# hby1320/pytorch_object_detection

Measured on AMD Instinct MI355X. Metric: images/sec HISFCOS-R50 640x640 inference, higher is better.
Workload: dtype f32

## Files before the change

include/fcosdet.h:

```cpp
#ifndef FCOSDET_H_
#define FCOSDET_H_

#include <stdint.h>

#ifdef __cplusplus
extern "C" {
#endif

#define FD_OK 0
#define FD_E_INVAL (-1)
#define FD_E_UNSUPPORTED (-2)
#define FD_E_LAUNCH (-3)

#define FD_MAX_SEG 8

#define FD_ACT_NONE 0
#define FD_ACT_RELU 1
#define FD_ACT_SILU 2
#define FD_ACT_EXP 3
#define FD_ACT_SIGMOID 4

typedef void* fd_stream_t;

typedef struct fd_segs {
// ... 55 lines not shown
    void* workspace;
    int64_t workspace_bytes;
    int32_t precision;
    int32_t res_mode;
    float seg_param[FD_MAX_SEG];
    fd_segs in;
    int32_t out_H, out_W;
    int32_t sc_sy, sc_sx, sc_oy, sc_ox, sc_H, sc_W;
    const float* gate;
    int32_t gate_cs;
    int32_t reserved0;
    const float* w_frag;
    float* gn_stats;
    int32_t gn_groups;
    int32_t gate_act;
    const float* gate_b;
    const float* x2;
    int32_t x2_cs, x2_co, x2_Cin, x2_stride, x2_H, x2_W;
    int32_t wg_first, wg_count;
    int32_t sk_wgs;
    int32_t io_f16;
} fd_conv_params;
int64_t fd_conv_sk_workspace_bytes(int32_t sk_wgs);

int32_t fd_conv2d_nhwc_f32(const fd_conv_params* p, fd_stream_t stream);
int32_t fd_conv_workgroups(const fd_conv_params* p);
int32_t fd_conv_workgroups_live(const fd_conv_params* p);
typedef struct fd_b2b_params {
    const float* x; const float* w1_frag; const float* scale1; const float* shift1; const float* res; float* y;
    const float* w2_frag; const float* scale2; const float* shift2; float* z;
    int32_t x_cs, x_co, res_cs, res_co, y_cs, y_co, z_cs, z_co;
    int32_t K1, N1, N2, act1, act2, reserved0;
    int64_t rows;
} fd_b2b_params;
int32_t fd_conv1x1_b2b_f32(const fd_b2b_params* p, fd_stream_t stream);
int32_t fd_conv_narrow_nco(int32_t Cout);
int64_t fd_conv_workspace_bytes(int64_t out_rows, int32_t Cout, int32_t ksplit);

int64_t fd_wino4_weight_bytes(int32_t N, int32_t K);
int32_t fd_wino4_pack_weights_f32(const float* w, const float* scale, float* out, int32_t Cout, int32_t Cin, int32_t mode, fd_stream_t stream);

int64_t fd_conv_weight_wave_bytes(int32_t Cout, int32_t Cin);
int32_t fd_pack_conv_weight_wave_f32(const float* w, float* out, int32_t Cout, int32_t Cin, fd_stream_t stream);

int64_t fd_wino_weight_bytes(int32_t Cout, int32_t Cin);
int32_t fd_wino_pack_weights_f32(const float* w, const float* scale, float* out, int32_t Cout, int32_t Cin, int32_t mode,
                                 fd_stream_t stream);

typedef struct fd_conv_wgrad_params {
    const float* x;
    const float* dy;
    float* dw;
    int32_t x_cs, x_co, dy_cs, dy_co;
    int32_t Cin, Cout, KH, KW, stride, pad, dil;
    void* workspace;
    int64_t workspace_bytes;
    int32_t nsplit;
    int32_t layout;
    const float* scale;
    fd_segs in;
    int32_t precision;
    int32_t io_f16;
} fd_conv_wgrad_params;

int64_t fd_conv_wgrad_workspace_bytes(int64_t out_rows, int32_t Cin, int32_t Cout, int32_t KH, int32_t KW);
int32_t fd_conv2d_bwd_weight_f32(const fd_conv_wgrad_params* p, fd_stream_t stream);
// ... 239 lines not shown
```

pytorch_object_detection_amd/_lib.py:

```python
from __future__ import annotations

import ctypes as C
import os

FD_MAX_SEG = 8
ACT_NONE, ACT_RELU, ACT_SILU, ACT_EXP, ACT_SIGMOID = 0, 1, 2, 3, 4
CONV_GENERIC, CONV_STEM = 0, 1
PREC_F32, PREC_F16X3, PREC_F16 = 0, 1, 2
TILES = {1: (128, 128), 2: (128, 64), 3: (64, 128), 4: (64, 64), 5: (128, 32), 6: (128, 96),
         7: (128, 128), 8: (128, 64), 9: (64, 128),
         10: (256, 128), 11: (256, 128),
         12: (128, 96),
         13: (128, 128),
         15: (64, 64)}
PATCH_TILE = 13
WAVE_TILE = 15
WINO_TILE = 14
WINO4_TILE = 16
NARROW_TILE = 17
F16K64_TILE = 18

_HERE = os.path.dirname(os.path.abspath(__file__))
LIB_PATH = os.environ.get("FD_LIB") or os.path.join(_HERE, "csrc", "libfcosdet_hip.so")

# ... 8 lines not shown
E_INVAL, E_UNSUPPORTED, E_LAUNCH = -1, -2, -3


class Segs(C.Structure):
    _fields_ = [("nseg", C.c_int32), ("batch", C.c_int32), ("H", C.c_int32 * FD_MAX_SEG), ("W", C.c_int32 * FD_MAX_SEG),
                ("m_start", C.c_int32 * (FD_MAX_SEG + 1))]

    @staticmethod
    def make(batch: int, hw) -> "Segs":
        s = Segs()
        s.nseg, s.batch = len(hw), batch
        m = 0
        for i, (h, w) in enumerate(hw):
            s.H[i], s.W[i], s.m_start[i] = h, w, m
            m += batch * h * w
        for i in range(len(hw), FD_MAX_SEG + 1):
            s.m_start[i] = m
        return s

    @property
    def rows(self) -> int:
        return self.m_start[self.nseg]

    def level_hw(self):
        return [(self.H[i], self.W[i]) for i in range(self.nseg)]


class B2BParams(C.Structure):
    _fields_ = [("x", C.c_void_p), ("w1_frag", C.c_void_p), ("scale1", C.c_void_p), ("shift1", C.c_void_p), ("res", C.c_void_p), ("y", C.c_void_p),
                ("w2_frag", C.c_void_p), ("scale2", C.c_void_p), ("shift2", C.c_void_p), ("z", C.c_void_p),
                ("x_cs", C.c_int32), ("x_co", C.c_int32), ("res_cs", C.c_int32), ("res_co", C.c_int32), ("y_cs", C.c_int32), ("y_co", C.c_int32),
                ("z_cs", C.c_int32), ("z_co", C.c_int32),
                ("K1", C.c_int32), ("N1", C.c_int32), ("N2", C.c_int32), ("act1", C.c_int32), ("act2", C.c_int32), ("reserved0", C.c_int32),
                ("rows", C.c_int64)]


class ConvParams(C.Structure):
    _fields_ = [("x", C.c_void_p), ("w", C.c_void_p), ("scale", C.c_void_p), ("shift", C.c_void_p), ("res", C.c_void_p),
                ("y", C.c_void_p),
                ("x_cs", C.c_int32), ("x_co", C.c_int32), ("res_cs", C.c_int32), ("res_co", C.c_int32),
                ("y_cs", C.c_int32), ("y_co", C.c_int32),
                ("Cin", C.c_int32), ("Cout", C.c_int32), ("KH", C.c_int32), ("KW", C.c_int32), ("stride", C.c_int32),
                ("pad", C.c_int32), ("dil", C.c_int32),
                ("act", C.c_int32), ("act_c0", C.c_int32), ("mode", C.c_int32), ("tile", C.c_int32), ("tag", C.c_int32), ("ksplit", C.c_int32),
                ("workspace", C.c_void_p), ("workspace_bytes", C.c_int64), ("precision", C.c_int32), ("res_mode", C.c_int32),
                ("seg_param", C.c_float * FD_MAX_SEG), ("segs", Segs),
                ("out_H", C.c_int32), ("out_W", C.c_int32), ("sc_sy", C.c_int32), ("sc_sx", C.c_int32), ("sc_oy", C.c_int32),
                ("sc_ox", C.c_int32), ("sc_H", C.c_int32), ("sc_W", C.c_int32),
                ("gate", C.c_void_p), ("gate_cs", C.c_int32), ("reserved0", C.c_int32), ("w_frag", C.c_void_p),
                ("gn_stats", C.c_void_p), ("gn_groups", C.c_int32), ("gate_act", C.c_int32), ("gate_b", C.c_void_p),
                ("x2", C.c_void_p), ("x2_cs", C.c_int32), ("x2_co", C.c_int32), ("x2_Cin", C.c_int32), ("x2_stride", C.c_int32), ("x2_H", C.c_int32),
                ("x2_W", C.c_int32), ("wg_first", C.c_int32), ("wg_count", C.c_int32), ("sk_wgs", C.c_int32), ("io_f16", C.c_int32)]


class PackJob(C.Structure):
    _fields_ = [("w", C.c_void_p), ("scale", C.c_void_p), ("out", C.c_void_p), ("Cout", C.c_int32), ("Cin", C.c_int32),
                ("KH", C.c_int32), ("KW", C.c_int32), ("mode", C.c_int32), ("reserved", C.c_int32)]


class WgradParams(C.Structure):
    _fields_ = [("x", C.c_void_p), ("dy", C.c_void_p), ("dw", C.c_void_p),
                ("x_cs", C.c_int32), ("x_co", C.c_int32), ("dy_cs", C.c_int32), ("dy_co", C.c_int32),
                ("Cin", C.c_int32), ("Cout", C.c_int32), ("KH", C.c_int32), ("KW", C.c_int32), ("stride", C.c_int32),
                ("pad", C.c_int32), ("dil", C.c_int32),
                ("workspace", C.c_void_p), ("workspace_bytes", C.c_int64), ("nsplit", C.c_int32), ("layout", C.c_int32),
                ("scale", C.c_void_p), ("segs", Segs), ("precision", C.c_int32), ("io_f16", C.c_int32)]

# ... 122 lines not shown
```

pytorch_object_detection_amd/csrc/fd_conv_b2b.hip:

```cpp
#include "fd_conv_common.h"

struct B2BArgs {
    const float* x; const float* res; float* y; float* z;
    const float* scale1; const float* shift1; const float* scale2; const float* shift2;
    int x_cs, x_co, res_cs, res_co, y_cs, y_co, z_cs, z_co;
    int M, KT1, NT1, N2, act1, act2;
    unsigned x_bytes, y_bytes, z_bytes, res_bytes;
};

template <int TM, int TN2>
__global__ __launch_bounds__(64, 2) void conv1x1_b2b_kernel(B2BArgs a, const float* __restrict__ wf1_, const float* __restrict__ wf2_) {
    extern __shared__ __attribute__((aligned(16))) char smem[];
    float* As = reinterpret_cast<float*>(smem);
    float* A2 = As + 32 * TM * 32;
    constexpr int NL = 4 * TM;
    const int lane = threadIdx.x, l31 = lane & 31, lh = lane >> 5;
    const int m0 = blockIdx.x * 32 * TM;

    constexpr unsigned OOB = 0xC0000000u;
    const __amdgpu_buffer_rsrc_t xrsrc = __builtin_amdgcn_make_buffer_rsrc((void*)a.x, (short)0, (int)a.x_bytes, 0x00020000);
    const int lrow = lane >> 3, chunk = lane & 7;
    unsigned a_off[NL];
#pragma unroll
    for (int i = 0; i < NL; ++i) {
        const int m = m0 + lrow + 8 * i;
        a_off[i] = (m < a.M) ? ((unsigned)m * (unsigned)a.x_cs + (unsigned)(a.x_co + chunk * 4)) * 4u : OOB;
    }
    const float4* __restrict__ wf1 = reinterpret_cast<const float4*>(wf1_) + lane;
    const float4* __restrict__ wf2 = reinterpret_cast<const float4*>(wf2_) + lane;
    const int KT1 = a.KT1, KT2 = 2 * a.NT1;

    float4 ra[NL];
    auto load_a = [&](int kt) {
        const unsigned kb = (unsigned)kt * 128u;
#pragma unroll
        for (int i = 0; i < NL; ++i)
            ra[i] = __builtin_bit_cast(float4, __builtin_amdgcn_raw_buffer_load_b128(xrsrc, (int)(a_off[i] + kb), 0, 0));
    };
    auto store_a = [&]() {
#pragma unroll
        for (int i = 0; i < NL; ++i) *reinterpret_cast<float4*>(As + lds_off(lrow + 8 * i, chunk)) = ra[i];
    };

    f32x16 acc2[TM][TN2];
#pragma unroll
    for (int i = 0; i < TM; ++i)
#pragma unroll
        for (int j = 0; j < TN2; ++j)
#pragma unroll
            for (int e = 0; e < 16; ++e) acc2[i][j][e] = 0.f;

    const int c4 = (lane & 7) * 4, prow = lane >> 3;
    float* stage = As;
    const __amdgpu_buffer_rsrc_t yrsrc = __builtin_amdgcn_make_buffer_rsrc((void*)a.y, (short)0, (int)a.y_bytes, 0x00020000);
    const __amdgpu_buffer_rsrc_t zrsrc = __builtin_amdgcn_make_buffer_rsrc((void*)a.z, (short)0, (int)a.z_bytes, 0x00020000);
    const __amdgpu_buffer_rsrc_t rrsrc = __builtin_amdgcn_make_buffer_rsrc((void*)(a.res ? a.res : a.x), (short)0, (int)a.res_bytes, 0x00020000);
    const unsigned y_off = ((unsigned)(m0 + prow) * (unsigned)a.y_cs + (unsigned)(a.y_co + c4)) * 4u;
    const unsigned z_off = ((unsigned)(m0 + prow) * (unsigned)a.z_cs + (unsigned)(a.z_co + c4)) * 4u;
    const unsigned r_off = ((unsigned)(m0 + prow) * (unsigned)a.res_cs + (unsigned)(a.res_co + c4)) * 4u;

    for (int n1t = 0; n1t < a.NT1; ++n1t) {
        f32x16 acc1[TM][2];
#pragma unroll
        for (int i = 0; i < TM; ++i)
#pragma unroll
            for (int j = 0; j < 2; ++j)
#pragma unroll
                for (int e = 0; e < 16; ++e) acc1[i][j][e] = 0.f;
        float4 fb[2][2];
        const float4* __restrict__ w1t = wf1 + (size_t)n1t * KT1 * 512;
        load_a(0);
#pragma unroll
        for (int j = 0; j < 2; ++j)
#pragma unroll
            for (int s = 0; s < 2; ++s) fb[j][s] = w1t[(j * 4 + s) * 64];
        for (int kt = 0; kt < KT1; ++kt) {
            store_a();
            __builtin_amdgcn_sched_barrier(0);
            if (kt + 1 < KT1) load_a(kt + 1);
            __builtin_amdgcn_sched_barrier(0);
            wave_lds_sync();
            const float4* __restrict__ wc_ = w1t + (size_t)kt * 512;
            const float4* __restrict__ wn_ = w1t + (size_t)min(kt + 1, KT1 - 1) * 512;
            __builtin_amdgcn_s_setprio(1);
#pragma unroll
            for (int s = 0; s < 4; ++s) {
                float4 fa[TM];
#pragma unroll
                for (int i = 0; i < TM; ++i) fa[i] = *reinterpret_cast<const float4*>(As + lds_off(i * 32 + l31, 2 * s + lh));
#pragma unroll
                for (int i = 0; i < TM; ++i)
#pragma unroll
// ... 11 lines not shown
            wave_lds_sync();
        }

#pragma unroll
        for (int j = 0; j < 2; ++j) {
            const int nb = n1t * 64 + 32 * j;
            const float sc = a.scale1 ? a.scale1[nb + l31] : 1.0f, sf = a.shift1 ? a.shift1[nb + l31] : 0.0f;
            float4 fb2[TN2][2];
            const int kt2 = 2 * n1t + j;
            auto w2at = [&](int jj, int s) { return wf2[((size_t)((jj >> 1) * KT2 + kt2) * 8 + (jj & 1) * 4 + s) * 64]; };
#pragma unroll
            for (int jj = 0; jj < TN2; ++jj)
#pragma unroll
                for (int s = 0; s < 2; ++s) fb2[jj][s] = w2at(jj, s);
#pragma unroll
            for (int i = 0; i < TM; ++i) {
                float4 rr[4];
#pragma unroll
                for (int p = 0; p < 4; ++p)
                    rr[p] = __builtin_bit_cast(float4, __builtin_amdgcn_raw_buffer_load_b128(rrsrc, (int)r_off, ((32 * i + 8 * p) * a.res_cs + nb) * 4, 0));
#pragma unroll
                for (int e = 0; e < 16; ++e) stage[((e & 3) + 8 * (e >> 2) + 4 * lh) * 32 + l31] = acc1[i][j][e] * sc + sf;
                wave_lds_sync();
#pragma unroll
                for (int p = 0; p < 4; ++p) {
                    float4 v = *reinterpret_cast<const float4*>(stage + (prow + 8 * p) * 32 + c4);
                    const float4 r = rr[p];
                    v.x += r.x; v.y += r.y; v.z += r.z; v.w += r.w;
                    if (a.act1 == FD_ACT_RELU) {
                        v.x = fmaxf(v.x, 0.f); v.y = fmaxf(v.y, 0.f); v.z = fmaxf(v.z, 0.f); v.w = fmaxf(v.w, 0.f);
                    } else if (a.act1 == FD_ACT_SILU) {
                        v.x = fd_act(v.x, FD_ACT_SILU, 0.f); v.y = fd_act(v.y, FD_ACT_SILU, 0.f); v.z = fd_act(v.z, FD_ACT_SILU, 0.f); v.w = fd_act(v.w, FD_ACT_SILU, 0.f);
                    }
                    __builtin_amdgcn_raw_buffer_store_b128(__builtin_bit_cast(f32x4, v), yrsrc, (int)y_off, ((32 * i + 8 * p) * a.y_cs + nb) * 4, 0);
                    *reinterpret_cast<float4*>(A2 + lds_off(32 * i + prow + 8 * p, lane & 7)) = v;
                }
                wave_lds_sync();
            }
            __builtin_amdgcn_s_setprio(1);
#pragma unroll
            for (int s = 0; s < 4; ++s) {
                float4 fa[TM];
#pragma unroll
                for (int i = 0; i < TM; ++i) fa[i] = *reinterpret_cast<const float4*>(A2 + lds_off(i * 32 + l31, 2 * s + lh));
#pragma unroll
                for (int i = 0; i < TM; ++i)
#pragma unroll
                    for (int jj = 0; jj < TN2; ++jj) {
                        acc2[i][jj] = __builtin_amdgcn_mfma_f32_32x32x2f32(fa[i].x, fb2[jj][s & 1].x, acc2[i][jj], 0, 0, 0);
                        acc2[i][jj] = __builtin_amdgcn_mfma_f32_32x32x2f32(fa[i].y, fb2[jj][s & 1].y, acc2[i][jj], 0, 0, 0);
                        acc2[i][jj] = __builtin_amdgcn_mfma_f32_32x32x2f32(fa[i].z, fb2[jj][s & 1].z, acc2[i][jj], 0, 0, 0);
                        acc2[i][jj] = __builtin_amdgcn_mfma_f32_32x32x2f32(fa[i].w, fb2[jj][s & 1].w, acc2[i][jj], 0, 0, 0);
                    }
                if (s < 2) {
#pragma unroll
                    for (int jj = 0; jj < TN2; ++jj) fb2[jj][s & 1] = w2at(jj, s + 2);
                }
                __builtin_amdgcn_sched_barrier(0);
            }
            __builtin_amdgcn_s_setprio(0);
            wave_lds_sync();
        }
    }

#pragma unroll
    for (int jj = 0; jj < TN2; ++jj) {
        const int nb = 32 * jj;
        if (nb >= a.N2) break;
        const float sc = a.scale2 ? a.scale2[nb + l31] : 1.0f, sf = a.shift2 ? a.shift2[nb + l31] : 0.0f;
#pragma unroll
        for (int i = 0; i < TM; ++i) {
#pragma unroll
            for (int e = 0; e < 16; ++e) stage[((e & 3) + 8 * (e >> 2) + 4 * lh) * 32 + l31] = acc2[i][jj][e] * sc + sf;
            wave_lds_sync();
#pragma unroll
            for (int p = 0; p < 4; ++p) {
                float4 v = *reinterpret_cast<const float4*>(stage + (prow + 8 * p) * 32 + c4);
                if (a.act2 == FD_ACT_RELU) {
                    v.x = fmaxf(v.x, 0.f); v.y = fmaxf(v.y, 0.f); v.z = fmaxf(v.z, 0.f); v.w = fmaxf(v.w, 0.f);
                } else if (a.act2 == FD_ACT_SILU) {
                    v.x = fd_act(v.x, FD_ACT_SILU, 0.f); v.y = fd_act(v.y, FD_ACT_SILU, 0.f); v.z = fd_act(v.z, FD_ACT_SILU, 0.f); v.w = fd_act(v.w, FD_ACT_SILU, 0.f);
                }
                __builtin_amdgcn_raw_buffer_store_b128(__builtin_bit_cast(f32x4, v), zrsrc, (int)z_off, ((32 * i + 8 * p) * a.z_cs + nb) * 4, 0);
            }
            wave_lds_sync();
        }
    }
}

extern "C" int32_t fd_conv1x1_b2b_f32(const fd_b2b_params* p, fd_stream_t stream_) {
    hipStream_t stream = (hipStream_t)stream_;
    FD_REQUIRE(p && p->x && p->w1_frag && p->w2_frag && p->y && p->z, FD_E_INVAL, "fd_conv1x1_b2b: null pointer");
    FD_REQUIRE(p->rows >= 1 && p->K1 >= 32 && p->K1 % 32 == 0 && p->N1 >= 64 && p->N1 % 64 == 0 && (p->N2 == 64 || p->N2 == 128), FD_E_UNSUPPORTED,
               "fd_conv1x1_b2b: needs K1 %% 32 == 0, N1 %% 64 == 0, N2 in {64, 128} (got %d -> %d -> %d)", p->K1, p->N1, p->N2);
    FD_REQUIRE(p->x_cs % 4 == 0 && p->x_co % 4 == 0 && p->x_cs >= p->x_co + p->K1 && p->y_cs % 4 == 0 && p->y_co % 4 == 0 && p->y_cs >= p->y_co + p->N1 &&
                   p->z_cs % 4 == 0 && p->z_co % 4 == 0 && p->z_cs >= p->z_co + p->N2 &&
                   (!p->res || (p->res_cs % 4 == 0 && p->res_co % 4 == 0 && p->res_cs >= p->res_co + p->N1)),
               FD_E_INVAL, "fd_conv1x1_b2b: channel views must be 4-aligned and in range");
    FD_REQUIRE((((uintptr_t)p->x | (uintptr_t)p->y | (uintptr_t)p->z | (uintptr_t)p->res | (uintptr_t)p->w1_frag | (uintptr_t)p->w2_frag) & 15) == 0, FD_E_INVAL,
               "fd_conv1x1_b2b: pointers must be 16-byte aligned");
    auto act_ok = [](int a_) { return a_ == FD_ACT_NONE || a_ == FD_ACT_RELU || a_ == FD_ACT_SILU; };
    FD_REQUIRE(act_ok(p->act1) && act_ok(p->act2), FD_E_UNSUPPORTED, "fd_conv1x1_b2b: activations none / ReLU / SiLU");
    const long xb = (long)p->rows * p->x_cs * 4;
    FD_REQUIRE(xb < 0xC0000000L - 65536 && (long)p->rows * p->y_cs * 4 < 0xC0000000L && (long)p->rows * p->z_cs * 4 < 0xC0000000L &&
                   (!p->res || (long)p->rows * p->res_cs * 4 < 0xC0000000L), FD_E_UNSUPPORTED, "fd_conv1x1_b2b: a view's buffer exceeds 3 GiB");
    B2BArgs a;
    a.x = p->x; a.res = p->res; a.y = p->y; a.z = p->z;
    a.scale1 = p->scale1; a.shift1 = p->shift1; a.scale2 = p->scale2; a.shift2 = p->shift2;
    a.x_cs = p->x_cs; a.x_co = p->x_co; a.res_cs = p->res_cs; a.res_co = p->res_co; a.y_cs = p->y_cs; a.y_co = p->y_co; a.z_cs = p->z_cs; a.z_co = p->z_co;
    a.M = (int)p->rows; a.KT1 = p->K1 / 32; a.NT1 = p->N1 / 64; a.N2 = p->N2; a.act1 = p->act1; a.act2 = p->act2;
    a.x_bytes = (unsigned)xb;
    a.y_bytes = (unsigned)((long)p->rows * p->y_cs * 4); a.z_bytes = (unsigned)((long)p->rows * p->z_cs * 4);
    a.res_bytes = p->res ? (unsigned)((long)p->rows * p->res_cs * 4) : 0u;
    if (p->N2 == 64) {
        const unsigned blocks = (unsigned)((p->rows + 63) / 64);
        hipLaunchKernelGGL((conv1x1_b2b_kernel<2, 2>), dim3(blocks), dim3(64), 2 * 64 * 32 * 4, stream, a, p->w1_frag, p->w2_frag);
    } else {
        const unsigned blocks = (unsigned)((p->rows + 31) / 32);
        hipLaunchKernelGGL((conv1x1_b2b_kernel<1, 4>), dim3(blocks), dim3(64), 2 * 32 * 32 * 4, stream, a, p->w1_frag, p->w2_frag);
    }
    FD_CHECK_LAUNCH("fd_conv1x1_b2b_f32");
    return FD_OK;
}
```

pytorch_object_detection_amd/engine.py:

```python
from __future__ import annotations

from typing import Callable, Dict, List, Optional, Sequence, Tuple

import torch

from . import ops
from . import _lib
from ._lib import ACT_EXP, ACT_NONE, ACT_RELU, ACT_SILU, FdError, Segs
from .ops import Rows


import os as _os

CONV_PRECISION = _os.environ.get("FD_CONV_PRECISION", "f32")
AUTOTUNE = True
GN_FUSED = _os.environ.get("FD_GN_FUSED", "1") != "0"
B2B_MIN_ROWS = 64 * 1024
B2B_LAYERS = "1"


class PRows(Rows):
    __slots__ = ("_flat",)


# ... 229 lines not shown
        plan.tail_steps = getattr(plan, "tail_steps", [])
        plan.tail_steps.append((name + ".tail", tail, 2 * out.rows * co * Cin * k * k - main_flops, dict(info)))
        return out
    plan.step_flops[len(plan.steps) - 1] = 2 * out.rows * co * Cin * k * k
    plan.step_info[len(plan.steps) - 1] = info
    return out


def add_input(plan: Plan, x4: Rows, batch: int, H: int, W: int, image_ref: List) -> None:
    mode = getattr(plan, "input_mode", None) or ("u8" if getattr(plan, "input_u8", None) else None)
    if mode == "u8":
        mean, std = plan.input_u8
        plan.add("input.preprocess_u8", lambda: ops.preprocess_u8(image_ref[0], x4.buf, mean, std))
    elif mode == "collate":
        mean, std = plan.input_u8
        hold = [None]

        def run():
            _, hold[0] = ops.collate_u8(image_ref[0], H, W, mean, std, out=x4.buf)
        plan.add("input.collate_u8", run)
    elif mode == "resize":
        mean, std = plan.input_u8
        hold = [None]
        plan.resized_hw = None
        plan.scales = torch.zeros(batch, dtype=torch.float32, device=plan.device)

        def run():
            _, hold[0] = ops.resize_collate_u8(image_ref[0], plan.resized_hw, H, W, mean, std, out=x4.buf)
        plan.add("input.resize_collate_u8", run)
    else:
        plan.add("input.nchw3_to_nhwc4", lambda: ops.nchw3_to_nhwc4(image_ref[0], x4.buf))


def build_resnet50(plan: Plan, trunk, batch: int, H: int, W: int, image_ref: List[torch.Tensor]):
    dev, pool = plan.device, plan.pool
    stem_own = plan.precision in ("f32", "mixed") and tuple(trunk.conv1.weight.shape) == (64, 3, 7, 7)
    mode = getattr(plan, "input_mode", None) or ("u8" if getattr(plan, "input_u8", None) else None)
    nchw_in = stem_own and mode is None
    x4 = None
    if not nchw_in:
        x4 = pool.get(batch * H * W, 4)
        add_input(plan, x4, batch, H, W, image_ref)
    s_in = Segs.make(batch, [(H, W)])
    sc, sf = ops.fold_bn(_dev(trunk.bn1.weight, dev), _dev(trunk.bn1.bias, dev), _dev(trunk.bn1.running_mean, dev),
                         _dev(trunk.bn1.running_var, dev), trunk.bn1.eps)
    s1 = ops.conv_out_segs(s_in, 7, 2, 3, 1)
    H1, W1 = s1.H[0], s1.W[0]
    H2, W2 = (H1 + 2 - 3) // 2 + 1, (W1 + 2 - 3) // 2 + 1
    s2 = Segs.make(batch, [(H2, W2)])

    def nchw_image() -> torch.Tensor:
        x = image_ref[0]
        if tuple(x.shape) != (batch, 3, H, W):
            raise FdError(f"plan input: expected a [{batch}, 3, {H}, {W}] batch, got {tuple(x.shape)}")
        return x

    y1 = None
    if stem_own:
        wp = ops.pack_stem7_weight(_dev(trunk.conv1.weight, dev))
        y2 = pool.get(s2.rows, 64)
        if nchw_in:
            plan.add("backbone.conv1+maxpool", lambda: ops.stem7x7_nchw(nchw_image(), wp, y2, sc, sf, pool=True))
        else:
            plan.add("backbone.conv1+maxpool", lambda: ops.stem7x7_pool(x4, wp, y2, batch, H, W, sc, sf))
    else:
        wp = ops.pack_stem_weight(_dev(trunk.conv1.weight, dev))
        y1 = pool.get(s1.rows, 64)
        plan.add("backbone.conv1", ops.conv_call(x4, s_in, wp, y1, Cin=4, Cout=64, k=7, stride=2, pad=3, scale=sc, shift=sf,
                                                 act=ACT_RELU, stem=True))
    plan.keep += [wp, sc, sf]
    plan.flops += 2 * s1.rows * 64 * 147
    plan.step_flops[len(plan.steps) - 1] = 2 * s1.rows * 64 * 147
    if x4 is not None:
        pool.put(x4)
    if y1 is not None:
        y2 = pool.get(s2.rows, 64)
        plan.add("backbone.maxpool", lambda: ops.maxpool(y1, y2, batch, H1, W1, 3, 2, 1))
        pool.put(y1)
    x, sx = y2, s2
    feats = []
    blocks_all = [(li, bi, blk) for li in (1, 2, 3, 4) for bi, blk in enumerate(getattr(trunk, f"layer{li}"))]
    o1_ready = None
    for gi, (li, bi, blk) in enumerate(blocks_all):
        nm = f"backbone.layer{li}.{bi}"
        planes = blk.conv1.weight.shape[0]
        so = ops.conv_out_segs(sx, 3, blk.conv2.stride[0], 1, 1)
        ds = blk.downsample
        if o1_ready is not None:
            o1, o1_ready = o1_ready, None
        else:
            o1 = pool.get(sx.rows, planes)
            add_conv(plan, nm + ".conv1", x, sx, blk.conv1, o1, bn=blk.bn1, act=ACT_RELU)
        o2 = pool.get(so.rows, planes)
        add_conv(plan, nm + ".conv2", o1, sx, blk.conv2, o2, bn=blk.bn2, act=ACT_RELU)
        pool.put(o1)
        dual = (ds is not None and plan.precision == "f32" and ds[0].kernel_size[0] == 1 and ds[0].bias is None and blk.conv3.bias is None
                and planes % 32 == 0 and x.C % 32 == 0 and x.cs % 4 == 0 and x.co % 4 == 0 and ds[0].stride[0] == blk.conv2.stride[0])
        if dual:
            f3 = ops.fold_bn(_dev(blk.bn3.weight, dev), _dev(blk.bn3.bias, dev), _dev(blk.bn3.running_mean, dev), _dev(blk.bn3.running_var, dev), blk.bn3.eps)
            fdn = ops.fold_bn(_dev(ds[1].weight, dev), _dev(ds[1].bias, dev), _dev(ds[1].running_mean, dev), _dev(ds[1].running_var, dev), ds[1].eps)
            wcat = torch.cat([_dev(blk.conv3.weight, dev) * f3[0][:, None, None, None], _dev(ds[0].weight, dev) * fdn[0][:, None, None, None]], 1)
            out = pool.get(so.rows, 4 * planes)
            add_conv(plan, nm + ".conv3+downsample", o2, so, blk.conv3, out, weight=wcat, fold=(None, (f3[1] + fdn[1]).contiguous()), act=ACT_RELU,
                     x2=x, x2_stride=ds[0].stride[0], x2_hw=(sx.H[0], sx.W[0]))
            plan.step_info[len(plan.steps) - 1]["dual"] = (planes, x.C, ds[0].stride[0])
            pool.put(o2)
            if not (feats and feats[-1][0] is x):
                pool.put(x)
            x, sx = out, so
            if li >= 2 and bi == len(getattr(trunk, f"layer{li}")) - 1:
                feats.append((x, sx))
            continue
        if ds is not None:
            idt = pool.get(so.rows, 4 * planes)
            add_conv(plan, nm + ".downsample", x, sx, ds[0], idt, bn=ds[1])
        else:
            idt = x
        out = pool.get(so.rows, 4 * planes)
        nxt = blocks_all[gi + 1][2] if gi + 1 < len(blocks_all) else None
        n2 = nxt.conv1.weight.shape[0] if nxt is not None else 0
        if (str(li) in B2B_LAYERS and so.rows >= B2B_MIN_ROWS and nxt is not None and plan.precision == "f32" and blk.conv3.bias is None and nxt.conv1.bias is None
                and nxt.conv1.kernel_size[0] == 1 and nxt.conv1.stride[0] == 1 and nxt.conv1.weight.shape[1] == 4 * planes
                and ops.b2b_ok(planes, 4 * planes, n2) and all(r.cs % 4 == 0 and r.co % 4 == 0 for r in (o2, out, idt))):
            o1_ready = pool.get(so.rows, n2)
            f3 = ops.fold_bn(_dev(blk.bn3.weight, dev), _dev(blk.bn3.bias, dev), _dev(blk.bn3.running_mean, dev), _dev(blk.bn3.running_var, dev), blk.bn3.eps)
            fn1 = ops.fold_bn(_dev(nxt.bn1.weight, dev), _dev(nxt.bn1.bias, dev), _dev(nxt.bn1.running_mean, dev), _dev(nxt.bn1.running_var, dev), nxt.bn1.eps)
            wa = ops.pack_conv_weight_wave(_dev(blk.conv3.weight, dev))
            wb = ops.pack_conv_weight_wave(_dev(nxt.conv1.weight, dev))
            plan.keep += [f3, fn1, wa, wb]
            nl, nb_ = blocks_all[gi + 1][0], blocks_all[gi + 1][1]
            plan.add(f"{nm}.conv3+layer{nl}.{nb_}.conv1",
                     ops.conv_b2b_call(o2, wa, out, wb, o1_ready, K1=planes, N1=4 * planes, N2=n2, scale1=f3[0], shift1=f3[1], res=idt, act1=ACT_RELU,
                                       scale2=fn1[0], shift2=fn1[1], act2=ACT_RELU))
            fl = 2 * so.rows * (4 * planes * planes + n2 * 4 * planes)
            plan.flops += fl
            plan.step_flops[len(plan.steps) - 1] = fl
            plan.step_info[len(plan.steps) - 1] = {"k": 1, "stride": 1, "dil": 1, "Cin": planes, "Cout": 4 * planes, "rows": so.rows, "family": "1x1",
                                                   "mfma_div": 1.0, "b2b": (4 * planes, n2)}
        else:
            add_conv(plan, nm + ".conv3", o2, so, blk.conv3, out, bn=blk.bn3, act=ACT_RELU, res=idt)
        pool.put(o2)
        if idt is not x:
            pool.put(idt)
        if not (feats and feats[-1][0] is x):
            pool.put(x)
        x, sx = out, so
        if li >= 2 and bi == len(getattr(trunk, f"layer{li}")) - 1:
            feats.append((x, sx))
    return feats


def build_efficientnet(plan: Plan, net, batch: int, H: int, W: int, image_ref: List[torch.Tensor], keep=(2, 3, 4)):
    dev, pool = plan.device, plan.pool
    x4 = pool.get(batch * H * W, 4)
    add_input(plan, x4, batch, H, W, image_ref)

    def out_hw(h: int, w: int, k: int, s: int, pad) -> Tuple[int, int]:
        return (h + pad[0] + pad[1] - k) // s + 1, (w + pad[0] + pad[1] - k) // s + 1

    def bn_fold(bn):
        sc, sf = ops.fold_bn(_dev(bn.weight, dev), _dev(bn.bias, dev), _dev(bn.running_mean, dev), _dev(bn.running_var, dev), bn.eps)
        plan.keep += [sc, sf]
        return sc, sf

    stem = net._conv_stem
    C0 = stem.weight.shape[0]
    h, w = out_hw(H, W, 3, 2, net.stem_pad)
    ws = ops.pack_stem3_weight(_dev(stem.weight, dev))
    sc0, sf0 = bn_fold(net._bn0)
    plan.keep.append(ws)
    x = pool.get(batch * h * w, C0)
    plan.add("backbone._conv_stem", lambda x=x, h=h, w=w: ops.stem_conv3(x4.buf, ws, x, batch, H, W, 3, 2, net.stem_pad[0], net.stem_pad[0],
                                                                       h, w, sc0, sf0, ACT_SILU))
    plan.flops += 2 * batch * h * w * C0 * 27
    pool.put(x4)
    blocks = list(net._blocks)
    ends: List[Optional[Tuple[Rows, Segs]]] = []
    for bi, blk in enumerate(blocks):
        nm = f"backbone._blocks.{bi}"
        segs = Segs.make(batch, [(h, w)])
# ... 507 lines not shown
```

pytorch_object_detection_amd/ops.py:

```python
from __future__ import annotations

import ctypes as C
import enum
import json
import math
import os
import re
from typing import Callable, List, NamedTuple, Optional, Sequence, Tuple

import numpy as np
import torch

from . import _lib
from ._lib import ACT_EXP, ACT_NONE, ACT_RELU, ACT_SIGMOID, ACT_SILU, ConvParams, FdError, Segs, check


CONV_LOG = None
LAUNCHES = [0]


def _stream() -> int:
    LAUNCHES[0] += 1
    return torch.cuda.current_stream().cuda_stream

# ... 272 lines not shown
                raise
            continue
        t = min(_time_launches(call, reps, False) for _ in range(3))
        if t < best_t * 0.98:
            best, best_t = wgs, t
    table[key] = best
    return best


def conv_workgroups(run) -> Tuple[int, int]:
    n = _lib.lib().fd_conv_workgroups(C.byref(run.params))
    live = _lib.lib().fd_conv_workgroups_live(C.byref(run.params))
    if n < 0 or live < 0:
        raise FdError("fd_conv_workgroups: " + _lib.lib().fd_last_error().decode(errors="replace"), int(min(n, live)))
    return (run.params.wg_count or n), live


def conv_wg_slice(run, first: int, count: int, tag: Optional[int] = None) -> Callable[[], None]:
    q = _lib.ConvParams()
    C.memmove(C.byref(q), C.byref(run.params), C.sizeof(q))
    q.wg_first, q.wg_count = first, count
    if tag is not None:
        q.tag = tag
    fn = _lib.lib().fd_conv2d_nhwc_f32
    ref = C.byref(q)

    def run_slice(_keep=(run, q)):
        check(fn(ref, _stream()), "fd_conv2d_nhwc_f32")

    run_slice.params = q
    return run_slice


def b2b_ok(K1: int, N1: int, N2: int) -> bool:
    return K1 % 32 == 0 and N1 % 64 == 0 and N2 in (64, 128)


def conv_b2b_call(x: Rows, w1_frag: torch.Tensor, y: Rows, w2_frag: torch.Tensor, z: Rows, *, K1: int, N1: int, N2: int,
                  scale1: Optional[torch.Tensor] = None, shift1: Optional[torch.Tensor] = None, res: Optional[Rows] = None, act1: int = ACT_NONE,
                  scale2: Optional[torch.Tensor] = None, shift2: Optional[torch.Tensor] = None, act2: int = ACT_NONE) -> Callable[[], None]:
    _need_gpu(w1_frag, w2_frag, scale1, shift1, scale2, shift2)
    p = _lib.B2BParams()
    p.x, p.w1_frag, p.y, p.w2_frag, p.z = x.ptr, w1_frag.data_ptr(), y.ptr, w2_frag.data_ptr(), z.ptr
    p.scale1 = scale1.data_ptr() if scale1 is not None else None
    p.shift1 = shift1.data_ptr() if shift1 is not None else None
    p.scale2 = scale2.data_ptr() if scale2 is not None else None
    p.shift2 = shift2.data_ptr() if shift2 is not None else None
    p.res = res.ptr if res is not None else None
    p.x_cs, p.x_co, p.y_cs, p.y_co, p.z_cs, p.z_co = x.cs, x.co, y.cs, y.co, z.cs, z.co
    if res is not None:
        p.res_cs, p.res_co = res.cs, res.co
    p.K1, p.N1, p.N2, p.act1, p.act2, p.rows = K1, N1, N2, act1, act2, y.rows
    fn = _lib.lib().fd_conv1x1_b2b_f32
    ref = C.byref(p)
    keep = (x, w1_frag, y, w2_frag, z, scale1, shift1, scale2, shift2, res, p)

    def run(_keep=keep):
        check(fn(ref, _stream()), "fd_conv1x1_b2b_f32")

    run.params = p
    return run


_TUNE_CACHE: dict = {}
_TUNE_FILE = os.environ.get("FD_TILE_TABLE") or os.path.join(os.path.dirname(os.path.abspath(__file__)), "tuned", "gfx950_tiles.json")
_TUNE_MODE = os.environ.get("FD_AUTOTUNE", "0")
_TUNE_LOADED = False


def _tune_table() -> dict:
    global _TUNE_LOADED
    if not _TUNE_LOADED:
        _TUNE_LOADED = True
        try:
            with open(_TUNE_FILE) as f:
                _TUNE_CACHE.update(json.load(f))
        except Exception:
            pass
    return _TUNE_CACHE


def save_tune_table() -> None:
    os.makedirs(os.path.dirname(_TUNE_FILE), exist_ok=True)
    with open(_TUNE_FILE, "w") as f:
        json.dump(dict(sorted(_TUNE_CACHE.items())), f, indent=0)


KSPLIT_MAX = 8
# ... 1225 lines not shown
```

Before: 1436.

## Extend back-to-back 1x1 kernel with dual-source K-concat and stride-2 compact output

Adds a second input source to the fused conv3+next-conv1 kernel, so the first block of a stage (conv3 plus downsample, K-concatenated) can also feed the next block's conv1 in one launch. It also lets the kernel store its block output only at even positions (a stride-2 compact map) when the only consumer is a stride-2 downsample. That consumer then reads the compact map at stride 1. The aim is fewer launches and less write and re-read traffic of large activation maps. In exchange it adds template variants, an LDS row-offset table, and a more complex graph-building path with new invariants.

```diff
diff --git a/include/fcosdet.h b/include/fcosdet.h
--- a/include/fcosdet.h
+++ b/include/fcosdet.h
@@ -111,6 +111,9 @@
     int32_t x_cs, x_co, res_cs, res_co, y_cs, y_co, z_cs, z_co;
     int32_t K1, N1, N2, act1, act2, reserved0;
     int64_t rows;
+    const float* x2;
+    int32_t x2_cs, x2_co, x2_K, x2_stride;
+    int32_t y_keep_stride, y_H, y_W, reserved1;
 } fd_b2b_params;
 int32_t fd_conv1x1_b2b_f32(const fd_b2b_params* p, fd_stream_t stream);
 int32_t fd_conv_narrow_nco(int32_t Cout);
diff --git a/pytorch_object_detection_amd/_lib.py b/pytorch_object_detection_amd/_lib.py
--- a/pytorch_object_detection_amd/_lib.py
+++ b/pytorch_object_detection_amd/_lib.py
@@ -64,7 +64,9 @@
                 ("x_cs", C.c_int32), ("x_co", C.c_int32), ("res_cs", C.c_int32), ("res_co", C.c_int32), ("y_cs", C.c_int32), ("y_co", C.c_int32),
                 ("z_cs", C.c_int32), ("z_co", C.c_int32),
                 ("K1", C.c_int32), ("N1", C.c_int32), ("N2", C.c_int32), ("act1", C.c_int32), ("act2", C.c_int32), ("reserved0", C.c_int32),
-                ("rows", C.c_int64)]
+                ("rows", C.c_int64),
+                ("x2", C.c_void_p), ("x2_cs", C.c_int32), ("x2_co", C.c_int32), ("x2_K", C.c_int32), ("x2_stride", C.c_int32),
+                ("y_keep_stride", C.c_int32), ("y_H", C.c_int32), ("y_W", C.c_int32), ("reserved1", C.c_int32)]
 
 
 class ConvParams(C.Structure):
diff --git a/pytorch_object_detection_amd/csrc/fd_conv_b2b.hip b/pytorch_object_detection_amd/csrc/fd_conv_b2b.hip
--- a/pytorch_object_detection_amd/csrc/fd_conv_b2b.hip
+++ b/pytorch_object_detection_amd/csrc/fd_conv_b2b.hip
@@ -5,14 +5,18 @@
     const float* scale1; const float* shift1; const float* scale2; const float* shift2;
     int x_cs, x_co, res_cs, res_co, y_cs, y_co, z_cs, z_co;
     int M, KT1, NT1, N2, act1, act2;
+    const float* x2; int x2_cs, x2_co, KTa;
+    int y_H, y_W;
+    unsigned x2_bytes;
     unsigned x_bytes, y_bytes, z_bytes, res_bytes;
 };
 
-template <int TM, int TN2>
+template <int TM, int TN2, bool DUAL, bool KEEP2>
 __global__ __launch_bounds__(64, 2) void conv1x1_b2b_kernel(B2BArgs a, const float* __restrict__ wf1_, const float* __restrict__ wf2_) {
     extern __shared__ __attribute__((aligned(16))) char smem[];
     float* As = reinterpret_cast<float*>(smem);
     float* A2 = As + 32 * TM * 32;
+    unsigned* Yo = reinterpret_cast<unsigned*>(A2 + 32 * TM * 32);
     constexpr int NL = 4 * TM;
     const int lane = threadIdx.x, l31 = lane & 31, lh = lane >> 5;
     const int m0 = blockIdx.x * 32 * TM;
@@ -26,12 +30,28 @@
         const int m = m0 + lrow + 8 * i;
         a_off[i] = (m < a.M) ? ((unsigned)m * (unsigned)a.x_cs + (unsigned)(a.x_co + chunk * 4)) * 4u : OOB;
     }
+    const __amdgpu_buffer_rsrc_t x2rsrc = __builtin_amdgcn_make_buffer_rsrc((void*)(DUAL ? a.x2 : a.x), (short)0, (int)(DUAL ? a.x2_bytes : 0u), 0x00020000);
+    unsigned a2_off[DUAL ? NL : 1];
+    if constexpr (DUAL) {
+#pragma unroll
+        for (int i = 0; i < NL; ++i) {
+            const int m = m0 + lrow + 8 * i;
+            a2_off[i] = (m < a.M) ? ((unsigned)m * (unsigned)a.x2_cs + (unsigned)(a.x2_co + chunk * 4)) * 4u : OOB;
+        }
+    }
     const float4* __restrict__ wf1 = reinterpret_cast<const float4*>(wf1_) + lane;
     const float4* __restrict__ wf2 = reinterpret_cast<const float4*>(wf2_) + lane;
     const int KT1 = a.KT1, KT2 = 2 * a.NT1;
 
     float4 ra[NL];
     auto load_a = [&](int kt) {
+        if (DUAL && kt >= a.KTa) {
+            const unsigned kb2 = (unsigned)(kt - a.KTa) * 128u;
+#pragma unroll
+            for (int i = 0; i < NL; ++i)
+                ra[i] = __builtin_bit_cast(float4, __builtin_amdgcn_raw_buffer_load_b128(x2rsrc, (int)(a2_off[DUAL ? i : 0] + kb2), 0, 0));
+            return;
+        }
         const unsigned kb = (unsigned)kt * 128u;
 #pragma unroll
         for (int i = 0; i < NL; ++i)
@@ -58,6 +78,17 @@
     const unsigned y_off = ((unsigned)(m0 + prow) * (unsigned)a.y_cs + (unsigned)(a.y_co + c4)) * 4u;
     const unsigned z_off = ((unsigned)(m0 + prow) * (unsigned)a.z_cs + (unsigned)(a.z_co + c4)) * 4u;
     const unsigned r_off = ((unsigned)(m0 + prow) * (unsigned)a.res_cs + (unsigned)(a.res_co + c4)) * 4u;
+    if constexpr (KEEP2) {
+        if (lane < 32 * TM) {
+            const int m = m0 + lane, hw = a.y_H * a.y_W;
+            const int n = m / hw, rem = m - n * hw;
+            const int h = rem / a.y_W, w = rem - h * a.y_W;
+            const int H2 = (a.y_H + 1) >> 1, W2 = (a.y_W + 1) >> 1;
+            const bool keep = m < a.M && !((h | w) & 1);
+            Yo[lane] = keep ? ((unsigned)((n * H2 + (h >> 1)) * W2 + (w >> 1)) * (unsigned)a.y_cs + (unsigned)a.y_co) * 4u : OOB;
+        }
+        wave_lds_sync();
+    }
 
     for (int n1t = 0; n1t < a.NT1; ++n1t) {
         f32x16 acc1[TM][2];
@@ -135,7 +166,10 @@
                     } else if (a.act1 == FD_ACT_SILU) {
                         v.x = fd_act(v.x, FD_ACT_SILU, 0.f); v.y = fd_act(v.y, FD_ACT_SILU, 0.f); v.z = fd_act(v.z, FD_ACT_SILU, 0.f); v.w = fd_act(v.w, FD_ACT_SILU, 0.f);
                     }
-                    __builtin_amdgcn_raw_buffer_store_b128(__builtin_bit_cast(f32x4, v), yrsrc, (int)y_off, ((32 * i + 8 * p) * a.y_cs + nb) * 4, 0);
+                    if constexpr (KEEP2)
+                        __builtin_amdgcn_raw_buffer_store_b128(__builtin_bit_cast(f32x4, v), yrsrc, (int)(Yo[32 * i + prow + 8 * p] + (unsigned)c4 * 4u), nb * 4, 0);
+                    else
+                        __builtin_amdgcn_raw_buffer_store_b128(__builtin_bit_cast(f32x4, v), yrsrc, (int)y_off, ((32 * i + 8 * p) * a.y_cs + nb) * 4, 0);
                     *reinterpret_cast<float4*>(A2 + lds_off(32 * i + prow + 8 * p, lane & 7)) = v;
                 }
                 wave_lds_sync();
@@ -189,6 +223,16 @@
             wave_lds_sync();
         }
     }
+}
+
+template <int TM, int TN2>
+static void b2b_launch(const B2BArgs& a, const fd_b2b_params* p, bool dual, bool keep2, hipStream_t stream) {
+    const unsigned blocks = (unsigned)((p->rows + 32 * TM - 1) / (32 * TM));
+    const size_t lds = 2 * 32 * TM * 32 * 4 + (keep2 ? 32 * TM * 4 : 0);
+    if (dual && keep2) hipLaunchKernelGGL((conv1x1_b2b_kernel<TM, TN2, true, true>), dim3(blocks), dim3(64), lds, stream, a, p->w1_frag, p->w2_frag);
+    else if (dual)     hipLaunchKernelGGL((conv1x1_b2b_kernel<TM, TN2, true, false>), dim3(blocks), dim3(64), lds, stream, a, p->w1_frag, p->w2_frag);
+    else if (keep2)    hipLaunchKernelGGL((conv1x1_b2b_kernel<TM, TN2, false, true>), dim3(blocks), dim3(64), lds, stream, a, p->w1_frag, p->w2_frag);
+    else               hipLaunchKernelGGL((conv1x1_b2b_kernel<TM, TN2, false, false>), dim3(blocks), dim3(64), lds, stream, a, p->w1_frag, p->w2_frag);
 }
 
 extern "C" int32_t fd_conv1x1_b2b_f32(const fd_b2b_params* p, fd_stream_t stream_) {
@@ -202,6 +246,21 @@
                FD_E_INVAL, "fd_conv1x1_b2b: channel views must be 4-aligned and in range");
     FD_REQUIRE((((uintptr_t)p->x | (uintptr_t)p->y | (uintptr_t)p->z | (uintptr_t)p->res | (uintptr_t)p->w1_frag | (uintptr_t)p->w2_frag) & 15) == 0, FD_E_INVAL,
                "fd_conv1x1_b2b: pointers must be 16-byte aligned");
+    const bool dual = p->x2 != nullptr, keep2 = p->y_keep_stride == 2;
+    if (dual) {
+        FD_REQUIRE(p->x2_stride == 1 && p->x2_K >= 32 && p->x2_K % 32 == 0, FD_E_UNSUPPORTED,
+                   "fd_conv1x1_b2b: the second source needs x2_stride == 1 and x2_K %% 32 == 0 (got stride %d, K %d)", p->x2_stride, p->x2_K);
+        FD_REQUIRE(p->x2_cs % 4 == 0 && p->x2_co % 4 == 0 && p->x2_cs >= p->x2_co + p->x2_K && ((uintptr_t)p->x2 & 15) == 0, FD_E_INVAL,
+                   "fd_conv1x1_b2b: the second source's channel view must be 4-aligned and in range, its pointer 16-byte aligned");
+        FD_REQUIRE((long)p->rows * p->x2_cs * 4 < 0xC0000000L - 65536, FD_E_UNSUPPORTED, "fd_conv1x1_b2b: a view's buffer exceeds 3 GiB");
+    }
+    FD_REQUIRE(p->y_keep_stride == 0 || p->y_keep_stride == 1 || keep2, FD_E_UNSUPPORTED, "fd_conv1x1_b2b: y_keep_stride 0 / 1 (every row) or 2 (got %d)", p->y_keep_stride);
+    long y_rows = p->rows;
+    if (keep2) {
+        FD_REQUIRE(p->y_H >= 1 && p->y_W >= 1 && (long)p->y_H * p->y_W <= p->rows && p->rows % ((long)p->y_H * p->y_W) == 0, FD_E_INVAL,
+                   "fd_conv1x1_b2b: y_keep_stride 2 needs rows = images * y_H * y_W (got %ld rows, %d x %d)", (long)p->rows, p->y_H, p->y_W);
+        y_rows = p->rows / ((long)p->y_H * p->y_W) * ((p->y_H + 1) / 2) * ((p->y_W + 1) / 2);
+    }
     auto act_ok = [](int a_) { return a_ == FD_ACT_NONE || a_ == FD_ACT_RELU || a_ == FD_ACT_SILU; };
     FD_REQUIRE(act_ok(p->act1) && act_ok(p->act2), FD_E_UNSUPPORTED, "fd_conv1x1_b2b: activations none / ReLU / SiLU");
     const long xb = (long)p->rows * p->x_cs * 4;
@@ -211,17 +270,14 @@
     a.x = p->x; a.res = p->res; a.y = p->y; a.z = p->z;
     a.scale1 = p->scale1; a.shift1 = p->shift1; a.scale2 = p->scale2; a.shift2 = p->shift2;
     a.x_cs = p->x_cs; a.x_co = p->x_co; a.res_cs = p->res_cs; a.res_co = p->res_co; a.y_cs = p->y_cs; a.y_co = p->y_co; a.z_cs = p->z_cs; a.z_co = p->z_co;
-    a.M = (int)p->rows; a.KT1 = p->K1 / 32; a.NT1 = p->N1 / 64; a.N2 = p->N2; a.act1 = p->act1; a.act2 = p->act2;
+    a.M = (int)p->rows; a.KT1 = (p->K1 + (dual ? p->x2_K : 0)) / 32; a.NT1 = p->N1 / 64; a.N2 = p->N2; a.act1 = p->act1; a.act2 = p->act2;
     a.x_bytes = (unsigned)xb;
-    a.y_bytes = (unsigned)((long)p->rows * p->y_cs * 4); a.z_bytes = (unsigned)((long)p->rows * p->z_cs * 4);
+    a.x2 = p->x2; a.x2_cs = p->x2_cs; a.x2_co = p->x2_co; a.KTa = p->K1 / 32; a.x2_bytes = dual ? (unsigned)((long)p->rows * p->x2_cs * 4) : 0u;
+    a.y_H = p->y_H; a.y_W = p->y_W;
+    a.y_bytes = (unsigned)(y_rows * p->y_cs * 4); a.z_bytes = (unsigned)((long)p->rows * p->z_cs * 4);
     a.res_bytes = p->res ? (unsigned)((long)p->rows * p->res_cs * 4) : 0u;
-    if (p->N2 == 64) {
-        const unsigned blocks = (unsigned)((p->rows + 63) / 64);
-        hipLaunchKernelGGL((conv1x1_b2b_kernel<2, 2>), dim3(blocks), dim3(64), 2 * 64 * 32 * 4, stream, a, p->w1_frag, p->w2_frag);
-    } else {
-        const unsigned blocks = (unsigned)((p->rows + 31) / 32);
-        hipLaunchKernelGGL((conv1x1_b2b_kernel<1, 4>), dim3(blocks), dim3(64), 2 * 32 * 32 * 4, stream, a, p->w1_frag, p->w2_frag);
-    }
+    if (p->N2 == 64) b2b_launch<2, 2>(a, p, dual, keep2, stream);
+    else b2b_launch<1, 4>(a, p, dual, keep2, stream);
     FD_CHECK_LAUNCH("fd_conv1x1_b2b_f32");
     return FD_OK;
 }
diff --git a/pytorch_object_detection_amd/engine.py b/pytorch_object_detection_amd/engine.py
--- a/pytorch_object_detection_amd/engine.py
+++ b/pytorch_object_detection_amd/engine.py
@@ -285,6 +285,20 @@
         plan.add("input.nchw3_to_nhwc4", lambda: ops.nchw3_to_nhwc4(image_ref[0], x4.buf))
 
 
+def _dual_ok(plan: Plan, blk, xC: int, xcs: int, xco: int) -> bool:
+    ds, planes = blk.downsample, blk.conv1.weight.shape[0]
+    return (ds is not None and plan.precision == "f32" and ds[0].kernel_size[0] == 1 and ds[0].bias is None and blk.conv3.bias is None
+            and planes % 32 == 0 and xC % 32 == 0 and xcs % 4 == 0 and xco % 4 == 0 and ds[0].stride[0] == blk.conv2.stride[0])
+
+
+def b2b_dual_ok(planes: int, x2_C: int, x2_stride: int, n2: int) -> bool:
+    return ops.b2b_ok(planes, 4 * planes, n2, x2_C, x2_stride)
+
+
+def y_compact_ok(readers: Sequence[tuple]) -> bool:
+    return list(readers) == [("x2", 2)]
+
+
 def build_resnet50(plan: Plan, trunk, batch: int, H: int, W: int, image_ref: List[torch.Tensor]):
     dev, pool = plan.device, plan.pool
     stem_own = plan.precision in ("f32", "mixed") and tuple(trunk.conv1.weight.shape) == (64, 3, 7, 7)
@@ -334,11 +348,40 @@
     feats = []
     blocks_all = [(li, bi, blk) for li in (1, 2, 3, 4) for bi, blk in enumerate(getattr(trunk, f"layer{li}"))]
     o1_ready = None
+    x_compact = False
     for gi, (li, bi, blk) in enumerate(blocks_all):
         nm = f"backbone.layer{li}.{bi}"
         planes = blk.conv1.weight.shape[0]
         so = ops.conv_out_segs(sx, 3, blk.conv2.stride[0], 1, 1)
         ds = blk.downsample
+        last = bi == len(getattr(trunk, f"layer{li}")) - 1
+        nxt = blocks_all[gi + 1][2] if gi + 1 < len(blocks_all) else None
+        n2 = nxt.conv1.weight.shape[0] if nxt is not None else 0
+        seam = (str(li) in B2B_LAYERS and so.rows >= B2B_MIN_ROWS and nxt is not None and plan.precision == "f32" and blk.conv3.bias is None and nxt.conv1.bias is None
+                and nxt.conv1.kernel_size[0] == 1 and nxt.conv1.stride[0] == 1 and nxt.conv1.weight.shape[1] == 4 * planes)
+        nl, nb_ = blocks_all[gi + 1][:2] if nxt is not None else (0, 0)
+
+        def b2b_step(name, x1, wcat, scale1, shift1, res, out, x2=None, keep2=False):
+            z = pool.get(so.rows, n2)
+            fn1 = ops.fold_bn(_dev(nxt.bn1.weight, dev), _dev(nxt.bn1.bias, dev), _dev(nxt.bn1.running_mean, dev), _dev(nxt.bn1.running_var, dev), nxt.bn1.eps)
+            wa = ops.pack_conv_weight_wave(wcat)
+            wb = ops.pack_conv_weight_wave(_dev(nxt.conv1.weight, dev))
+            plan.keep += [scale1, shift1, fn1, wa, wb]
+            plan.add(name, ops.conv_b2b_call(x1, wa, out, wb, z, K1=planes, N1=4 * planes, N2=n2, scale1=scale1, shift1=shift1, res=res, act1=ACT_RELU,
+                                             scale2=fn1[0], shift2=fn1[1], act2=ACT_RELU, x2=x2, x2_stride=1,
+                                             y_keep_stride=2 if keep2 else 1, y_hw=(so.H[0], so.W[0]) if keep2 else None))
+            fl = 2 * so.rows * (4 * planes * wcat.shape[1] + n2 * 4 * planes)
+            plan.flops += fl
+            plan.step_flops[len(plan.steps) - 1] = fl
+            info = {"k": 1, "stride": 1, "dil": 1, "Cin": planes, "Cout": 4 * planes, "rows": so.rows, "family": "1x1", "mfma_div": 1.0, "b2b": (4 * planes, n2),
+                    "y_rows": out.rows}
+            if x2 is not None:
+                info["dual"] = (planes, x2.C, 1)
+            plan.step_info[len(plan.steps) - 1] = info
+            return z
+
+        if x_compact and o1_ready is None:
+            raise FdError(f"{nm}: its input map was stored at stride 2, but its conv1 has not been computed by the producer")
         if o1_ready is not None:
             o1, o1_ready = o1_ready, None
         else:
@@ -347,21 +390,31 @@
         o2 = pool.get(so.rows, planes)
         add_conv(plan, nm + ".conv2", o1, sx, blk.conv2, o2, bn=blk.bn2, act=ACT_RELU)
         pool.put(o1)
-        dual = (ds is not None and plan.precision == "f32" and ds[0].kernel_size[0] == 1 and ds[0].bias is None and blk.conv3.bias is None
-                and planes % 32 == 0 and x.C % 32 == 0 and x.cs % 4 == 0 and x.co % 4 == 0 and ds[0].stride[0] == blk.conv2.stride[0])
+        dual = _dual_ok(plan, blk, x.C, x.cs, x.co)
+        if x_compact and not (dual and ds[0].stride[0] == 2):
+            raise FdError(f"{nm}: its input map was stored at stride 2 for a stride-2 K-concatenated GEMM, which this block does not end in")
         if dual:
             f3 = ops.fold_bn(_dev(blk.bn3.weight, dev), _dev(blk.bn3.bias, dev), _dev(blk.bn3.running_mean, dev), _dev(blk.bn3.running_var, dev), blk.bn3.eps)
             fdn = ops.fold_bn(_dev(ds[1].weight, dev), _dev(ds[1].bias, dev), _dev(ds[1].running_mean, dev), _dev(ds[1].running_var, dev), ds[1].eps)
             wcat = torch.cat([_dev(blk.conv3.weight, dev) * f3[0][:, None, None, None], _dev(ds[0].weight, dev) * fdn[0][:, None, None, None]], 1)
             out = pool.get(so.rows, 4 * planes)
-            add_conv(plan, nm + ".conv3+downsample", o2, so, blk.conv3, out, weight=wcat, fold=(None, (f3[1] + fdn[1]).contiguous()), act=ACT_RELU,
-                     x2=x, x2_stride=ds[0].stride[0], x2_hw=(sx.H[0], sx.W[0]))
-            plan.step_info[len(plan.steps) - 1]["dual"] = (planes, x.C, ds[0].stride[0])
+            shift = (f3[1] + fdn[1]).contiguous()
+            if (seam and not x_compact and b2b_dual_ok(planes, x.C, ds[0].stride[0], n2)
+                    and all(r.cs % 4 == 0 and r.co % 4 == 0 for r in (o2, out, x))):
+                o1_ready = b2b_step(f"{nm}.conv3+downsample+layer{nl}.{nb_}.conv1", o2, wcat, None, shift, None, out, x2=x)
+            elif x_compact:
+                add_conv(plan, nm + ".conv3+downsample", o2, so, blk.conv3, out, weight=wcat, fold=(None, shift), act=ACT_RELU,
+                         x2=x, x2_stride=1, x2_hw=((sx.H[0] + 1) // 2, (sx.W[0] + 1) // 2))
+                plan.step_info[len(plan.steps) - 1]["dual"] = (planes, x.C, ds[0].stride[0])
+            else:
+                add_conv(plan, nm + ".conv3+downsample", o2, so, blk.conv3, out, weight=wcat, fold=(None, shift), act=ACT_RELU,
+                         x2=x, x2_stride=ds[0].stride[0], x2_hw=(sx.H[0], sx.W[0]))
+                plan.step_info[len(plan.steps) - 1]["dual"] = (planes, x.C, ds[0].stride[0])
             pool.put(o2)
             if not (feats and feats[-1][0] is x):
                 pool.put(x)
-            x, sx = out, so
-            if li >= 2 and bi == len(getattr(trunk, f"layer{li}")) - 1:
+            x, sx, x_compact = out, so, False
+            if li >= 2 and last:
                 feats.append((x, sx))
             continue
         if ds is not None:
@@ -369,36 +422,26 @@
             add_conv(plan, nm + ".downsample", x, sx, ds[0], idt, bn=ds[1])
         else:
             idt = x
-        out = pool.get(so.rows, 4 * planes)
-        nxt = blocks_all[gi + 1][2] if gi + 1 < len(blocks_all) else None
-        n2 = nxt.conv1.weight.shape[0] if nxt is not None else 0
-        if (str(li) in B2B_LAYERS and so.rows >= B2B_MIN_ROWS and nxt is not None and plan.precision == "f32" and blk.conv3.bias is None and nxt.conv1.bias is None
-                and nxt.conv1.kernel_size[0] == 1 and nxt.conv1.stride[0] == 1 and nxt.conv1.weight.shape[1] == 4 * planes
-                and ops.b2b_ok(planes, 4 * planes, n2) and all(r.cs % 4 == 0 and r.co % 4 == 0 for r in (o2, out, idt))):
-            o1_ready = pool.get(so.rows, n2)
+        keep2 = False
+        if seam and ops.b2b_ok(planes, 4 * planes, n2) and all(r.cs % 4 == 0 and r.co % 4 == 0 for r in (o2, idt)):
+            nxt_dual = _dual_ok(plan, nxt, 4 * planes, 4 * planes, 0)
+            readers = [("x2", nxt.downsample[0].stride[0])] if nxt_dual else [("downsample",) if nxt.downsample is not None else ("identity",)]
+            if li >= 2 and last:
+                readers.append(("feature",))
+            keep2 = so.nseg == 1 and y_compact_ok(readers)
+            out = pool.get(batch * ((so.H[0] + 1) // 2) * ((so.W[0] + 1) // 2) if keep2 else so.rows, 4 * planes)
             f3 = ops.fold_bn(_dev(blk.bn3.weight, dev), _dev(blk.bn3.bias, dev), _dev(blk.bn3.running_mean, dev), _dev(blk.bn3.running_var, dev), blk.bn3.eps)
-            fn1 = ops.fold_bn(_dev(nxt.bn1.weight, dev), _dev(nxt.bn1.bias, dev), _dev(nxt.bn1.running_mean, dev), _dev(nxt.bn1.running_var, dev), nxt.bn1.eps)
-            wa = ops.pack_conv_weight_wave(_dev(blk.conv3.weight, dev))
-            wb = ops.pack_conv_weight_wave(_dev(nxt.conv1.weight, dev))
-            plan.keep += [f3, fn1, wa, wb]
-            nl, nb_ = blocks_all[gi + 1][0], blocks_all[gi + 1][1]
-            plan.add(f"{nm}.conv3+layer{nl}.{nb_}.conv1",
-                     ops.conv_b2b_call(o2, wa, out, wb, o1_ready, K1=planes, N1=4 * planes, N2=n2, scale1=f3[0], shift1=f3[1], res=idt, act1=ACT_RELU,
-                                       scale2=fn1[0], shift2=fn1[1], act2=ACT_RELU))
-            fl = 2 * so.rows * (4 * planes * planes + n2 * 4 * planes)
-            plan.flops += fl
-            plan.step_flops[len(plan.steps) - 1] = fl
-            plan.step_info[len(plan.steps) - 1] = {"k": 1, "stride": 1, "dil": 1, "Cin": planes, "Cout": 4 * planes, "rows": so.rows, "family": "1x1",
-                                                   "mfma_div": 1.0, "b2b": (4 * planes, n2)}
+            o1_ready = b2b_step(f"{nm}.conv3+layer{nl}.{nb_}.conv1", o2, _dev(blk.conv3.weight, dev), f3[0], f3[1], idt, out, keep2=keep2)
         else:
+            out = pool.get(so.rows, 4 * planes)
             add_conv(plan, nm + ".conv3", o2, so, blk.conv3, out, bn=blk.bn3, act=ACT_RELU, res=idt)
         pool.put(o2)
         if idt is not x:
             pool.put(idt)
         if not (feats and feats[-1][0] is x):
             pool.put(x)
-        x, sx = out, so
-        if li >= 2 and bi == len(getattr(trunk, f"layer{li}")) - 1:
+        x, sx, x_compact = out, so, keep2
+        if li >= 2 and last:
             feats.append((x, sx))
     return feats
 
diff --git a/pytorch_object_detection_amd/ops.py b/pytorch_object_detection_amd/ops.py
--- a/pytorch_object_detection_amd/ops.py
+++ b/pytorch_object_detection_amd/ops.py
@@ -328,14 +328,23 @@
     return run_slice
 
 
-def b2b_ok(K1: int, N1: int, N2: int) -> bool:
-    return K1 % 32 == 0 and N1 % 64 == 0 and N2 in (64, 128)
+def b2b_ok(K1: int, N1: int, N2: int, x2_K: int = 0, x2_stride: int = 1) -> bool:
+    return K1 >= 32 and K1 % 32 == 0 and N1 % 64 == 0 and N2 in (64, 128) and x2_K % 32 == 0 and (x2_K == 0 or x2_stride == 1)
 
 
 def conv_b2b_call(x: Rows, w1_frag: torch.Tensor, y: Rows, w2_frag: torch.Tensor, z: Rows, *, K1: int, N1: int, N2: int,
                   scale1: Optional[torch.Tensor] = None, shift1: Optional[torch.Tensor] = None, res: Optional[Rows] = None, act1: int = ACT_NONE,
-                  scale2: Optional[torch.Tensor] = None, shift2: Optional[torch.Tensor] = None, act2: int = ACT_NONE) -> Callable[[], None]:
+                  scale2: Optional[torch.Tensor] = None, shift2: Optional[torch.Tensor] = None, act2: int = ACT_NONE,
+                  x2: Optional[Rows] = None, x2_stride: int = 1, y_keep_stride: int = 1, y_hw: Optional[Tuple[int, int]] = None) -> Callable[[], None]:
     _need_gpu(w1_frag, w2_frag, scale1, shift1, scale2, shift2)
+    rows = z.rows
+    if y_keep_stride == 2:
+        if y_hw is None or y_hw[0] < 1 or y_hw[1] < 1 or rows % (y_hw[0] * y_hw[1]):
+            raise FdError("conv_b2b_call: y_keep_stride = 2 needs y_hw = (H, W) with rows = images * H * W")
+        if y.rows != rows // (y_hw[0] * y_hw[1]) * ((y_hw[0] + 1) // 2) * ((y_hw[1] + 1) // 2):
+            raise FdError("conv_b2b_call: the compact y map must hold images * ceil(H / 2) * ceil(W / 2) rows")
+    elif y.rows != rows:
+        raise FdError("conv_b2b_call: y and z must have the same number of rows")
     p = _lib.B2BParams()
     p.x, p.w1_frag, p.y, p.w2_frag, p.z = x.ptr, w1_frag.data_ptr(), y.ptr, w2_frag.data_ptr(), z.ptr
     p.scale1 = scale1.data_ptr() if scale1 is not None else None
@@ -346,10 +355,15 @@
     p.x_cs, p.x_co, p.y_cs, p.y_co, p.z_cs, p.z_co = x.cs, x.co, y.cs, y.co, z.cs, z.co
     if res is not None:
         p.res_cs, p.res_co = res.cs, res.co
-    p.K1, p.N1, p.N2, p.act1, p.act2, p.rows = K1, N1, N2, act1, act2, y.rows
+    p.K1, p.N1, p.N2, p.act1, p.act2, p.rows = K1, N1, N2, act1, act2, rows
+    if x2 is not None:
+        p.x2, p.x2_cs, p.x2_co, p.x2_K, p.x2_stride = x2.ptr, x2.cs, x2.co, x2.C, x2_stride
+    p.y_keep_stride = y_keep_stride
+    if y_hw is not None:
+        p.y_H, p.y_W = y_hw
     fn = _lib.lib().fd_conv1x1_b2b_f32
     ref = C.byref(p)
-    keep = (x, w1_frag, y, w2_frag, z, scale1, shift1, scale2, shift2, res, p)
+    keep = (x, w1_frag, y, w2_frag, z, scale1, shift1, scale2, shift2, res, p, x2)
 
     def run(_keep=keep):
         check(fn(ref, _stream()), "fd_conv1x1_b2b_f32")
```

Result: no change. 1440 (median of 6 runs) (+0.3%).
